# Jimmy2027/MoPoE-MIMIC

Hardware: AMD Instinct MI355X
Metric: samples/sec (higher is better)
Workload: dtype f32; 1 GPU; BASELINE config c2: MoPoE joint-ELBO train step, 3 modalities (PA+Lateral+text) 128x128, class_dim 128, DIM_img 64, DIM_text 128, vocab 3517, batch 64/GPU, fp32 (storage, accumulation and every product; where the launch plan says so the fp32 products are formed on the bf16 matrix pipe from exact three-way splits of both operands -- closer to fp64 than the fp32 MFMA, tests: test_f32_products_on_the; global_batch=64, parallelism=dp1, hip_graph=True, cross_rank_elbo=mean

## Files before the change

mopoe-mimic_amd/csrc/conv_gemm.hip:

```cpp
#include "gemm_common.hpp"

namespace mopoe {

#ifndef GEMM_MIN_WAVES
#define GEMM_MIN_WAVES 3
#endif
#ifndef GEMM_LDS_PAD
#define GEMM_LDS_PAD 4
#endif
constexpr int LDS_PAD = GEMM_LDS_PAD;

struct GemmArgs {
  const float* X;
  const float* W;
  float* Y;
  const float* bias;
  int N, Hx, Wx, Hy, Wy, Ck, Cn, Cin_w, Cout_w;
  int kh, kw, sh, sw, ph, pw;
  int form, w_nk;
  int Hq, Wq;
  long rows_per_phase;
  int vecA, vecB;
  mopoe_bn_ref bn_in;
  mopoe_mask_ref mask;
  double* out_stats;
  mopoe_bn_ref relu_bn;
  const float* xin;
  double* bwd_sums;
  unsigned x_bytes, w_bytes;
  int nsplit;
  float* partial;
  int* counters;
  long rows_total;
  int mix;
  float mix_a, mix_b;
  int xcd_remap;
};

__device__ __forceinline__ float epi_round(const GemmArgs&, float x) { return x; }
struct EpiXinRaw { float4 lo, hi; };
constexpr bool EPI_PREFETCH_XIN = false;
__device__ __forceinline__ EpiXinRaw epi_xin_ld(const GemmArgs& a, long yrow, int ncol, bool ok_hi) {
  const float* p = a.xin + yrow * a.Cn + ncol;
// ... 6 lines not shown
  xi[0] = r.lo.x; xi[1] = r.lo.y; xi[2] = r.lo.z; xi[3] = r.lo.w; xi[4] = r.hi.x; xi[5] = r.hi.y; xi[6] = r.hi.z; xi[7] = r.hi.w;
}
__device__ __forceinline__ void epi_store8(const GemmArgs& a, long yrow, int ncol, bool ok_hi, const float (&v)[8]) {
  float* dst = a.Y + yrow * a.Cn + ncol;
  *reinterpret_cast<float4*>(dst) = make_float4(v[0], v[1], v[2], v[3]);
  if (ok_hi) *reinterpret_cast<float4*>(dst + 4) = make_float4(v[4], v[5], v[6], v[7]);
}


__device__ __forceinline__ float4 bld4(__amdgpu_buffer_rsrc_t srd, unsigned byte_off) {
  const u32x4 v = __builtin_amdgcn_raw_buffer_load_b128(srd, byte_off, 0, 0);
  return make_float4(__uint_as_float(v.x), __uint_as_float(v.y), __uint_as_float(v.z), __uint_as_float(v.w));
}

__device__ __forceinline__ float4 bld4s(__amdgpu_buffer_rsrc_t srd, unsigned byte_off, unsigned s_off) {
  const u32x4 v = __builtin_amdgcn_raw_buffer_load_b128(srd, byte_off, s_off, 0);
  return make_float4(__uint_as_float(v.x), __uint_as_float(v.y), __uint_as_float(v.z), __uint_as_float(v.w));
}

__device__ __forceinline__ float4 ld4(const float* p, int nvalid, bool vec) {
  float4 v = make_float4(0.f, 0.f, 0.f, 0.f);
  if (nvalid >= 4 && vec) {
    v = *reinterpret_cast<const float4*>(p);
  } else {
    if (nvalid > 0) v.x = p[0];
    if (nvalid > 1) v.y = p[1];
    if (nvalid > 2) v.z = p[2];
    if (nvalid > 3) v.w = p[3];
  }
  return v;
}

template <int BM, int BN, int WGM, int WGN, int GBK, bool VEC, int SPEC = 0>
__global__ __launch_bounds__(64 * WGM * WGN, (WGM * WGN == 4 ? GEMM_MIN_WAVES : ((BM / WGM) * (BN / WGN) > 64 * 32 ? 2 : 4)))
void gather_gemm_kernel(const GemmArgs a) {
  static_assert(SPEC == 0 || VEC, "specialised loops exist for the vector path only");
  constexpr int NT = 64 * WGM * WGN;
  static_assert(WGM * WGN == 4 || WGM * WGN == 8, "4 or 8 waves per block");
  constexpr int WM = BM / WGM, WN = BN / WGN;
  constexpr int TI = WM / 32, TJ = WN / 32;
  constexpr int A_LD = BM + LDS_PAD, B_LD = BN + LDS_PAD;
  constexpr int KQ = GBK / 4;
  constexpr int RPP = NT / KQ;
  constexpr int A_PER_THR = BM / RPP;
  static_assert(BM % RPP == 0, "A tile rows must be a multiple of the rows covered per pass");
  constexpr int B_PER_THR_NK = (BN + RPP - 1) / RPP;
  constexpr int N4 = BN / 4;
  constexpr int B_PER_THR_KN = (GBK * N4 + NT - 1) / NT;
  constexpr int B_PER_THR = B_PER_THR_NK > B_PER_THR_KN ? B_PER_THR_NK : B_PER_THR_KN;

  constexpr int STG_LD = WN + 4;
  constexpr int A_FLOATS = 2 * GBK * A_LD, B_FLOATS = 2 * GBK * B_LD;
  constexpr int STG_FLOATS = VEC ? (NT / 64) * 32 * STG_LD : 0;
  constexpr int SMEM_FLOATS = (A_FLOATS + B_FLOATS) > STG_FLOATS ? (A_FLOATS + B_FLOATS) : STG_FLOATS;
  __shared__ __attribute__((aligned(16))) float smem[SMEM_FLOATS];
  __shared__ __attribute__((aligned(16))) float bnS[MAX_BN_C];
  __shared__ __attribute__((aligned(16))) float bnT[MAX_BN_C];
  __shared__ __attribute__((aligned(16))) float epi[5][VEC ? BN : 4];
  __shared__ int s_ticket;
  float* const As0 = smem;
  float* const Bs0 = smem + A_FLOATS;
#define AS_(buf, k, r) As0[((buf) * GBK + (k)) * A_LD + (r)]
#define BS_(buf, k, r) Bs0[((buf) * GBK + (k)) * B_LD + (r)]

  const int tid = threadIdx.x;
  const int lane = tid & 63, wave = tid >> 6;
  const int wm = wave / WGN, wn = wave % WGN;
  unsigned lbx = blockIdx.x, lby = blockIdx.y, lbz = blockIdx.z;
  if (a.xcd_remap) {
    const unsigned inner = gridDim.y * gridDim.z;
    const unsigned sw = xcd_swizzle(blockIdx.x + gridDim.x * (blockIdx.y + gridDim.y * blockIdx.z), gridDim.x * inner);
    lbx = sw / inner;
    const unsigned rem = sw - lbx * inner;
    lby = rem % gridDim.y;
    lbz = rem / gridDim.y;
  }
  const int n0 = lby * BN;
  const int phase = lbz / a.nsplit;
  const int split = lbz - phase * a.nsplit;

  const TapWalk tw = tap_walk(a, phase);
  const int nty = tw.nty, ntx = tw.ntx, ky0 = tw.ky0, kx0 = tw.kx0, kstep_y = tw.kstep_y, kstep_x = tw.kstep_x;
// ... 65 lines not shown
    for (int i = 0; i < B_PER_THR_KN; ++i) {
      const int k = tid / N4 + i * (NT / N4);
      const int n = n0 + (tid % N4) * 4;
      if ((k < GBK) & (n < a.Cn)) voffB[i] = ((unsigned)k * (unsigned)a.Cout_w + (unsigned)n) * 4u;
    }
  } else {
#pragma unroll
    for (int i = 0; i < B_PER_THR_NK; ++i) {
      const int n = n0 + trow + i * RPP;
      if ((trow + i * RPP < BN) & (n < a.Cn)) voffB[i] = ((unsigned)n * (unsigned)a.Cout_w + (unsigned)kq * 4u) * 4u;
    }
  }

  const long nMt = (a.rows_per_phase + BM - 1) / BM;
  for (long mt = lbx; mt < nMt; mt += gridDim.x) {
    const long m0 = mt * BM;

    int rn[A_PER_THR], ry0[A_PER_THR], rx0[A_PER_THR], rbase[A_PER_THR];
    bool rvalid[A_PER_THR];
#pragma unroll
    for (int i = 0; i < A_PER_THR; ++i) {
      const long m = m0 + trow + i * RPP;
      rvalid[i] = m < a.rows_per_phase;
      const unsigned mm = rvalid[i] ? (unsigned)m : 0u;
      const int n = (int)(mm / (unsigned)hw);
      const int rem = (int)(mm - (unsigned)n * (unsigned)hw);
      const int qy = rem / a.Wq, qx = rem - qy * a.Wq;
      rn[i] = n;
      if (a.form == 0) { ry0[i] = qy * a.sh - a.ph; rx0[i] = qx * a.sw - a.pw; }
      else             { ry0[i] = qy + cy;          rx0[i] = qx + cx; }
      rbase[i] = (n * a.Hx + ry0[i]) * a.Wx + rx0[i];
    }

    float4 ra[A_PER_THR], rb[B_PER_THR];
    float4 pend_sc = make_float4(0.f, 0.f, 0.f, 0.f), pend_sh = pend_sc;
    bool pend_ok[A_PER_THR];

    int ld_tap = it_beg / nkc;
    int ld_kc = (it_beg - ld_tap * nkc) * GBK;
    bool tap_dirty = true;
    unsigned offA[A_PER_THR], offW = 0;
    bool okA[A_PER_THR];

    auto load_tiles = [&](int ) {
      if (tap_dirty) {
        const int jy = ld_tap / ntx, jx = ld_tap - jy * ntx;
        const int wtap = (ky0 + kstep_y * jy) * a.kw + (kx0 + kstep_x * jx);
        const int tapoff = dsgn * (jy * a.Wx + jx);
#pragma unroll
        for (int i = 0; i < A_PER_THR; ++i) {
          const int iy = ry0[i] + dsgn * jy, ix = rx0[i] + dsgn * jx;
          okA[i] = rvalid[i] & ((unsigned)iy < (unsigned)a.Hx) & ((unsigned)ix < (unsigned)a.Wx);
          offA[i] = (unsigned)(rbase[i] + tapoff) * (unsigned)a.Ck * 4u;
        }
        offW = (unsigned)wtap * (unsigned)a.Cin_w * (unsigned)a.Cout_w * 4u;
        if (fastk) {
#pragma unroll
          for (int i = 0; i < A_PER_THR; ++i) {
            offA[i] = okA[i] ? offA[i] + (unsigned)kq * 16u : OOB;
            pend_ok[i] = okA[i];
          }
        }
        tap_dirty = false;
      }
      if (fastk) {
        const unsigned sA = (unsigned)ld_kc * 4u;
        const unsigned sB = offW + (w_nk == 0 ? (unsigned)ld_kc * (unsigned)a.Cout_w * 4u : (unsigned)ld_kc * 4u);
        if (xform) {
          pend_sc = *reinterpret_cast<const float4*>(&bnS[ld_kc + kq * 4]);
          pend_sh = *reinterpret_cast<const float4*>(&bnT[ld_kc + kq * 4]);
        }
        if constexpr (VEC) {
#pragma unroll
          for (int i = 0; i < A_PER_THR; ++i) ra[i] = bld4s(srdX, offA[i], sA);
          if (w_nk == 0) {
#pragma unroll
            for (int i = 0; i < B_PER_THR_KN; ++i) rb[i] = bld4s(srdW, voffB[i], sB);
          } else {
#pragma unroll
            for (int i = 0; i < B_PER_THR_NK; ++i) rb[i] = bld4s(srdW, voffB[i], sB);
          }
        }
        ld_kc += GBK;
        if (ld_kc >= nkc * GBK) { ld_kc = 0; ++ld_tap; tap_dirty = true; }
        return;
      }
      const int kc = ld_kc;
      const int ck = kc + kq * 4;
      const int nvk = a.Ck - ck;
      if (xform) {
        const int cks = nvk > 0 ? ck : 0;
        pend_sc = *reinterpret_cast<const float4*>(&bnS[cks]);
        pend_sh = *reinterpret_cast<const float4*>(&bnT[cks]);
      }
#pragma unroll
      for (int i = 0; i < A_PER_THR; ++i) {
        const bool ok = okA[i] & (nvk > 0);
        float4 v;
        if constexpr (VEC) {
          v = bld4(srdX, ok ? offA[i] + (unsigned)ck * 4u : OOB);
        } else {
          v = make_float4(0.f, 0.f, 0.f, 0.f);
          if (ok) v = ld4(a.X + (long)(offA[i] >> 2) + ck, nvk, false);
        }
        pend_ok[i] = ok;
        ra[i] = v;
      }
      if (w_nk == 0) {
#pragma unroll
        for (int i = 0; i < B_PER_THR_KN; ++i) {
          const int k = tid / N4 + i * (NT / N4);
          const int n = n0 + (tid % N4) * 4;
          const int kk = kc + k;
          const bool ok = (k < GBK) & (kk < a.Ck) & (n < a.Cn);
          if constexpr (VEC) {
            rb[i] = bld4(srdW, ok ? offW + ((unsigned)kk * (unsigned)a.Cout_w + (unsigned)n) * 4u : OOB);
          } else {
            float4 v = make_float4(0.f, 0.f, 0.f, 0.f);
            if (ok) v = ld4(a.W + (long)(offW >> 2) + (long)kk * a.Cout_w + n, a.Cn - n, false);
            rb[i] = v;
          }
        }
      } else {
#pragma unroll
        for (int i = 0; i < B_PER_THR_NK; ++i) {
          const int n = n0 + trow + i * RPP;
          const bool ok = (trow + i * RPP < BN) & (n < a.Cn) & (nvk > 0);
          if constexpr (VEC) {
            rb[i] = bld4(srdW, ok ? offW + ((unsigned)n * (unsigned)a.Cout_w + (unsigned)ck) * 4u : OOB);
          } else {
            float4 v = make_float4(0.f, 0.f, 0.f, 0.f);
            if (ok) v = ld4(a.W + (long)(offW >> 2) + (long)n * a.Cout_w + ck, nvk, false);
            rb[i] = v;
          }
        }
      }
      ld_kc += GBK;
      if (ld_kc >= nkc * GBK) { ld_kc = 0; ++ld_tap; tap_dirty = true; }
    };

    auto store_tiles = [&](auto bufc) {
      constexpr int buf = decltype(bufc)::value;
#pragma unroll
      for (int i = 0; i < A_PER_THR; ++i) {
        const int r = trow + i * RPP;
        if (xform) {
          const bool ok = pend_ok[i];
          ra[i].x = ok ? fmaxf(fmaf(ra[i].x, pend_sc.x, pend_sh.x), 0.f) : 0.f;
          ra[i].y = ok ? fmaxf(fmaf(ra[i].y, pend_sc.y, pend_sh.y), 0.f) : 0.f;
          ra[i].z = ok ? fmaxf(fmaf(ra[i].z, pend_sc.z, pend_sh.z), 0.f) : 0.f;
          ra[i].w = ok ? fmaxf(fmaf(ra[i].w, pend_sc.w, pend_sh.w), 0.f) : 0.f;
        }
        AS_(buf, kq * 4 + 0, r) = ra[i].x;
        AS_(buf, kq * 4 + 1, r) = ra[i].y;
        AS_(buf, kq * 4 + 2, r) = ra[i].z;
        AS_(buf, kq * 4 + 3, r) = ra[i].w;
      }
      if (w_nk == 0) {
#pragma unroll
        for (int i = 0; i < B_PER_THR_KN; ++i) {
          const int k = tid / N4 + i * (NT / N4);
          if (k < GBK) *reinterpret_cast<float4*>(&BS_(buf, k, (tid % N4) * 4)) = rb[i];
        }
      } else {
#pragma unroll
        for (int i = 0; i < B_PER_THR_NK; ++i) {
          const int r = trow + i * RPP;
          if (r >= BN) continue;
          BS_(buf, kq * 4 + 0, r) = rb[i].x;
          BS_(buf, kq * 4 + 1, r) = rb[i].y;
          BS_(buf, kq * 4 + 2, r) = rb[i].z;
          BS_(buf, kq * 4 + 3, r) = rb[i].w;
        }
      }
    };

    f32x16 acc[TI][TJ];
#pragma unroll
    for (int i = 0; i < TI; ++i)
#pragma unroll
      for (int j = 0; j < TJ; ++j)
#pragma unroll
        for (int r = 0; r < 16; ++r) acc[i][j][r] = 0.f;

    if (total > 0) {
      load_tiles(it_beg);
      store_tiles(std::integral_constant<int, 0>{});
    }
    __syncthreads();

    auto chunk = [&](int it, auto curc) {
      constexpr int cur = decltype(curc)::value;
      if (it + 1 < total) load_tiles(it_beg + it + 1);
      __builtin_amdgcn_sched_barrier(0);
#ifdef GEMM_SETPRIO
      __builtin_amdgcn_s_setprio(1);
#endif
#pragma unroll
      for (int kk = 0; kk < GBK / 2; ++kk) {
        const int k = kk * 2 + lhi;
        float av[TI], bv[TJ];
#pragma unroll
        for (int i = 0; i < TI; ++i) av[i] = AS_(cur, k, wm * WM + i * 32 + l31);
#pragma unroll
        for (int j = 0; j < TJ; ++j) bv[j] = BS_(cur, k, wn * WN + j * 32 + l31);
#pragma unroll
        for (int i = 0; i < TI; ++i)
#pragma unroll
          for (int j = 0; j < TJ; ++j)
            acc[i][j] = __builtin_amdgcn_mfma_f32_32x32x2f32(av[i], bv[j], acc[i][j], 0, 0, 0);
      }
#ifdef GEMM_SETPRIO
      __builtin_amdgcn_s_setprio(0);
#endif
      if (it + 1 < total) store_tiles(std::integral_constant<int, cur ^ 1>{});
      __syncthreads();
    };
    int it = 0;
    for (; it + 1 < total; it += 2) {
      chunk(it, std::integral_constant<int, 0>{});
      chunk(it + 1, std::integral_constant<int, 1>{});
    }
    if (it < total) chunk(it, std::integral_constant<int, 0>{});

    if constexpr (VEC) {
#include "gemm_epilogue_rows.inc"
    } else {
#include "gemm_epilogue.inc"
    }
  }

  if constexpr (VEC) {
#include "gemm_colstats_rows.inc"
  } else {
#include "gemm_colstats.inc"
  }
#undef AS_
#undef BS_
}

__device__ __forceinline__ float bld1s(__amdgpu_buffer_rsrc_t srd, unsigned byte_off, unsigned s_off) {
  return __uint_as_float(__builtin_amdgcn_raw_buffer_load_b32(srd, byte_off, s_off, 0));
}

template <int WGM, int WGN, int TI, int TJ, int SPEC>
__global__ __launch_bounds__(64 * WGM * WGN, (TI * TJ >= 4 ? 3 : 4)) void direct_gemm_kernel(const GemmArgs a) {
  constexpr int NT = 64 * WGM * WGN;
  constexpr int WM = TI * 32, WN = TJ * 32, BM = WGM * WM, BN = WGN * WN;
  constexpr bool xform = SPEC == 2;
  constexpr int w_nk = SPEC == 3 ? 1 : 0;
  constexpr int KS = 8;

  __shared__ __attribute__((aligned(16))) float bnS[xform ? MAX_BN_C : 4];
  __shared__ __attribute__((aligned(16))) float bnT[xform ? MAX_BN_C : 4];

  const int tid = threadIdx.x;
// ... 202 lines not shown
  __shared__ __attribute__((aligned(16))) float Is[2][BK][I_LD];
  __shared__ __attribute__((aligned(16))) float Js[2][BK][J_LD];
  __shared__ __attribute__((aligned(16))) float bnS[MAX_BN_C];
  __shared__ __attribute__((aligned(16))) float bnT[MAX_BN_C];

  const int tid = threadIdx.x;
  const int lane = tid & 63, wave = tid >> 6;
  const int wi = wave >> 1, wj = wave & 1;
  const unsigned lin = a.xcd_remap ? xcd_swizzle(blockIdx.x + gridDim.x * (blockIdx.y + gridDim.y * blockIdx.z),
                                                 gridDim.x * gridDim.y * gridDim.z)
                                   : blockIdx.x + gridDim.x * (blockIdx.y + gridDim.y * blockIdx.z);
  const unsigned bx = lin % gridDim.x, byz = lin / gridDim.x;
  const unsigned by = byz % gridDim.y, bz = byz / gridDim.y;
  const int it_i = bx / a.nJ, it_j = bx % a.nJ;
  const int i0 = it_i * BI, j0 = it_j * BJ;
  const int tap = by;
  const int ky = tap / a.kw, kx = tap % a.kw;
  const long mbeg = (long)bz * a.chunk;
  const long mend = mbeg + a.chunk < a.Ms ? mbeg + a.chunk : a.Ms;
  const int total = (int)((mend - mbeg + BK - 1) / BK);

  const bool xform = SPEC ? (SPEC == 2) : (a.bn_in.mode != 0);
  const bool fast = SPEC ? true : (VEC && a.fast != 0);
  if (xform) {
    for (int c = tid; c < ((a.Cin + 3) & ~3); c += 256) {
      BnC k = BnC{0.f, 0.f, 0.f, 0.f};
      if (c < a.Cin) k = bn_coef(a.bn_in, c);
      bnS[c] = k.scale;
      bnT[c] = k.shift;
    }
    __syncthreads();
  }

  float4 ri[I_PER_THR], rj[J_PER_THR];
  bool pend_ok[I_PER_THR];
  const int hw = a.Hs * a.Ws;
  const __amdgpu_buffer_rsrc_t srdX = __builtin_amdgcn_make_buffer_rsrc((void*)a.Xs, 0, (int)a.x_bytes, 0x00020000);
  const __amdgpu_buffer_rsrc_t srdD = __builtin_amdgcn_make_buffer_rsrc((void*)a.Dy, 0, (int)a.dy_bytes, 0x00020000);

  static_assert(BI == BJ, "both operand tiles cover the same pixels per thread");
  constexpr int PPP = 256 / I4;
  int pn[I_PER_THR], pqy[I_PER_THR], pqx[I_PER_THR];
  long pm[I_PER_THR];
#pragma unroll
  for (int t = 0; t < I_PER_THR; ++t) {
    pm[t] = mbeg + tid / I4 + t * PPP;
    const unsigned m = (unsigned)(pm[t] < a.Ms ? pm[t] : 0);
    const unsigned n = m / (unsigned)hw;
    const unsigned rem = m - n * (unsigned)hw;
    pn[t] = (int)n; pqy[t] = rem / a.Ws; pqx[t] = rem - pqy[t] * a.Ws;
  }

  float4 sc4 = make_float4(0.f, 0.f, 0.f, 0.f), sh4 = sc4;
  const int ci = i0 + (tid % I4) * 4, cj = j0 + (tid % J4) * 4;
  if (xform) {
    const int cs = ci < a.Cin ? ci : 0;
    sc4 = *reinterpret_cast<const float4*>(&bnS[cs]);
    sh4 = *reinterpret_cast<const float4*>(&bnT[cs]);
  }

  const int rpc = a.Ws >= BK ? 1 : BK / a.Ws;
  const int big_c = a.x_is_big ? a.Cin : a.Cout;
  const unsigned shift_rows = (unsigned)(a.ph * a.Wb + a.pw);
  const unsigned shift_bytes = shift_rows * (unsigned)big_c * 4u;
  const __amdgpu_buffer_rsrc_t srdBig = __builtin_amdgcn_make_buffer_rsrc(
      (void*)((const char*)(a.x_is_big ? a.Xs : a.Dy) - shift_bytes), 0,
      (int)((a.x_is_big ? a.x_bytes : a.dy_bytes) + shift_bytes), 0x00020000);
  int f_ly[I_PER_THR], f_lx[I_PER_THR];
  unsigned f_vbig[I_PER_THR], f_vsmall_i[I_PER_THR], f_vsmall_j[I_PER_THR];
  int f_slot[I_PER_THR];
  int f_n = 0, f_qy = 0, f_qx = 0;
  unsigned f_m0 = 0;
  if (fast) {
#pragma unroll
    for (int t = 0; t < I_PER_THR; ++t) {
      const int p = tid / I4 + t * PPP;
      const int pdy = a.Ws >= BK ? 0 : p / a.Ws, pqx = a.Ws >= BK ? p : p - (p / a.Ws) * a.Ws;
      f_slot[t] = p;
      f_ly[t] = pdy * a.sh + ky - a.ph;
      f_lx[t] = pqx * a.sw + kx - a.pw;
      const unsigned lane_rows = (unsigned)((f_ly[t] + a.ph) * a.Wb + (f_lx[t] + a.pw));
      const int cbig = a.x_is_big ? ci : cj;
      f_vbig[t] = (cbig < big_c) ? (lane_rows * (unsigned)big_c + (unsigned)cbig) * 4u : OOB;
      f_vsmall_i[t] = (ci < a.Cin) ? ((unsigned)p * (unsigned)a.Cin + (unsigned)ci) * 4u : OOB;
      f_vsmall_j[t] = (cj < a.Cout) ? ((unsigned)p * (unsigned)a.Cout + (unsigned)cj) * 4u : OOB;
    }
    const unsigned m0 = (unsigned)mbeg;
    f_m0 = m0;
    f_n = (int)(m0 / (unsigned)hw);
    const unsigned rem = m0 - (unsigned)f_n * (unsigned)hw;
    f_qy = (int)(rem / (unsigned)a.Ws);
    f_qx = (int)(rem - (unsigned)f_qy * (unsigned)a.Ws);
  }

  auto load_tiles = [&](int ) {
    if (fast) {
      if constexpr (VEC) {
        const int nleft = (int)((unsigned)mend - f_m0);
        const int s_by = f_qy * a.sh, s_bx = f_qx * a.sw;
        const unsigned s_big = (unsigned)((f_n * a.Hb + s_by) * a.Wb + s_bx) * (unsigned)big_c * 4u;
        const unsigned s_small_i = f_m0 * (unsigned)a.Cin * 4u, s_small_j = f_m0 * (unsigned)a.Cout * 4u;
#pragma unroll
        for (int t = 0; t < I_PER_THR; ++t) {
          const bool inm = f_slot[t] < nleft;
          const bool inb = ((unsigned)(s_by + f_ly[t]) < (unsigned)a.Hb) & ((unsigned)(s_bx + f_lx[t]) < (unsigned)a.Wb);
          const unsigned vb = (inm & inb) ? f_vbig[t] : OOB;
          if (a.x_is_big) {
            ri[t] = bld4s(srdBig, vb, s_big);
            rj[t] = bld4s(srdD, inm ? f_vsmall_j[t] : OOB, s_small_j);
            pend_ok[t] = (inm & inb) & (ci < a.Cin);
          } else {
            ri[t] = bld4s(srdX, inm ? f_vsmall_i[t] : OOB, s_small_i);
            rj[t] = bld4s(srdBig, vb, s_big);
            pend_ok[t] = inm & (ci < a.Cin);
          }
        }
        f_m0 += BK;
        if (a.Ws >= BK) { f_qx += BK; if (f_qx >= a.Ws) { f_qx = 0; ++f_qy; } }
        else f_qy += rpc;
        if (f_qy >= a.Hs) { f_qy = 0; ++f_n; }
      }
      return;
    }
#pragma unroll
    for (int t = 0; t < I_PER_THR; ++t) {
      const bool inm = pm[t] < mend;
      const int by = pqy[t] * a.sh - a.ph + ky, bx = pqx[t] * a.sw - a.pw + kx;
      const bool inb = ((unsigned)by < (unsigned)a.Hb) & ((unsigned)bx < (unsigned)a.Wb);
      const int srow = (int)pm[t];
      const int brow = (pn[t] * a.Hb + by) * a.Wb + bx;
      const int rowx = a.x_is_big ? brow : srow, rowd = a.x_is_big ? srow : brow;
      const bool okx = inm & (ci < a.Cin) & (a.x_is_big ? inb : true);
      const bool okd = inm & (cj < a.Cout) & (a.x_is_big ? true : inb);
      pend_ok[t] = okx;
      if constexpr (VEC) {
        ri[t] = bld4(srdX, okx ? ((unsigned)rowx * (unsigned)a.Cin + (unsigned)ci) * 4u : OOB);
        rj[t] = bld4(srdD, okd ? ((unsigned)rowd * (unsigned)a.Cout + (unsigned)cj) * 4u : OOB);
      } else {
        float4 v = make_float4(0.f, 0.f, 0.f, 0.f), w = v;
        if (okx) v = ld4(a.Xs + (long)rowx * a.Cin + ci, a.Cin - ci, false);
        if (okd) w = ld4(a.Dy + (long)rowd * a.Cout + cj, a.Cout - cj, false);
        ri[t] = v; rj[t] = w;
      }
      pm[t] += BK;
      pqx[t] += BK;
      if (pqx[t] >= a.Ws) {
        if (a.Ws >= BK) {
          pqx[t] -= a.Ws; ++pqy[t];
        } else {
          const int carry = pqx[t] / a.Ws;
          pqx[t] -= carry * a.Ws; pqy[t] += carry;
        }
        if (pqy[t] >= a.Hs) {
          const int carry = pqy[t] / a.Hs;
          pqy[t] -= carry * a.Hs; pn[t] += carry;
        }
      }
    }
  };

  auto store_tiles = [&](auto bufc) {
    constexpr int buf = decltype(bufc)::value;
#pragma unroll
    for (int t = 0; t < I_PER_THR; ++t) {
      const int p = tid / I4 + t * (256 / I4);
      if (xform) {
        const bool ok = pend_ok[t];
        ri[t].x = ok ? fmaxf(fmaf(ri[t].x, sc4.x, sh4.x), 0.f) : 0.f;
        ri[t].y = ok ? fmaxf(fmaf(ri[t].y, sc4.y, sh4.y), 0.f) : 0.f;
        ri[t].z = ok ? fmaxf(fmaf(ri[t].z, sc4.z, sh4.z), 0.f) : 0.f;
        ri[t].w = ok ? fmaxf(fmaf(ri[t].w, sc4.w, sh4.w), 0.f) : 0.f;
      }
      *reinterpret_cast<float4*>(&Is[buf][p][(tid % I4) * 4]) = ri[t];
    }
#pragma unroll
    for (int t = 0; t < J_PER_THR; ++t) {
      const int p = tid / J4 + t * (256 / J4);
      *reinterpret_cast<float4*>(&Js[buf][p][(tid % J4) * 4]) = rj[t];
    }
  };

  f32x16 acc[TI][TJ];
#pragma unroll
  for (int i = 0; i < TI; ++i)
#pragma unroll
    for (int j = 0; j < TJ; ++j)
#pragma unroll
      for (int r = 0; r < 16; ++r) acc[i][j][r] = 0.f;

  if (total > 0) {
    load_tiles(0);
    store_tiles(std::integral_constant<int, 0>{});
  }
  __syncthreads();

  const int l31 = lane & 31, lhi = lane >> 5;
  auto chunk = [&](int it, auto curc) {
    constexpr int cur = decltype(curc)::value;
    if (it + 1 < total) load_tiles(it + 1);
    __builtin_amdgcn_sched_barrier(0);
#pragma unroll
    for (int kk = 0; kk < BK / 2; ++kk) {
      const int k = kk * 2 + lhi;
      float av[TI], bv[TJ];
#pragma unroll
      for (int i = 0; i < TI; ++i) av[i] = Is[cur][k][wi * WI + i * 32 + l31];
#pragma unroll
      for (int j = 0; j < TJ; ++j) bv[j] = Js[cur][k][wj * WJ + j * 32 + l31];
#pragma unroll
      for (int i = 0; i < TI; ++i)
#pragma unroll
        for (int j = 0; j < TJ; ++j)
          acc[i][j] = __builtin_amdgcn_mfma_f32_32x32x2f32(av[i], bv[j], acc[i][j], 0, 0, 0);
    }
    if (it + 1 < total) store_tiles(std::integral_constant<int, cur ^ 1>{});
    __syncthreads();
  };
  int it = 0;
  for (; it + 1 < total; it += 2) {
    chunk(it, std::integral_constant<int, 0>{});
    chunk(it + 1, std::integral_constant<int, 1>{});
  }
  if (it < total) chunk(it, std::integral_constant<int, 0>{});

#pragma unroll
  for (int j = 0; j < TJ; ++j) {
    const int co = j0 + wj * WJ + j * 32 + l31;
    if (co >= a.Cout) continue;
#pragma unroll
    for (int i = 0; i < TI; ++i) {
#pragma unroll
      for (int r = 0; r < 16; ++r) {
        const int ci = i0 + wi * WI + i * 32 + (r & 3) + 8 * (r >> 2) + 4 * lhi;
        if (ci >= a.Cin) continue;
        float* dst = a.dW + ((long)tap * a.Cin + ci) * a.Cout + co;
        if (a.atomic) unsafeAtomicAdd(dst, acc[i][j][r]);
        else *dst = acc[i][j][r];
      }
    }
  }
}

#ifndef EPI_MAX_BLOCKS_Y
#define EPI_MAX_BLOCKS_Y 256
#endif
__global__ __launch_bounds__(256) void splitk_epilogue_kernel(const GemmArgs a) {
  __shared__ float cs[2][4][64];
  const int tx = threadIdx.x & 63, ty = threadIdx.x >> 6;
  const int n = blockIdx.x * 64 + tx;
  const bool nok = n < a.Cn;
  const bool do_relu_bn = a.relu_bn.mode != 0;
  const float bias = (nok && a.bias) ? a.bias[n] : 0.f;
  BnC rb = {0.f, 0.f, 0.f, 0.f};
  if (nok && do_relu_bn) rb = bn_coef(a.relu_bn, n);
  const long stride = a.rows_total * (long)a.Cn;
  float s1 = 0.f, s2 = 0.f;
// ... 214 lines not shown
```

mopoe-mimic_amd/csrc/gemm_common.hpp:

```cpp
#pragma once
#include <stdlib.h>
#include <algorithm>
#include <initializer_list>
#include <type_traits>

#include "common.hpp"
#include "conv_launch.hpp"

namespace mopoe {

bool edge_supported(const mopoe_conv_geom* g, int C, std::initializer_list<const void*> ptrs);
template <typename T> int edge_expand(const float* scal, const float* W, T* out, const mopoe_conv_geom* g, int C, double* stats, hipStream_t st);
template <typename T> int edge_wgrad(const T* vec, const float* scal, float* dW, const mopoe_conv_geom* g, int C, hipStream_t st, bool dw_is_zero = false);
template <typename T> int edge_reduce(const T* x, const float* W, const float* bias, float* out, const mopoe_conv_geom* g, int C, hipStream_t st);

typedef float f32x16 __attribute__((ext_vector_type(16)));
typedef unsigned int u32x4 __attribute__((ext_vector_type(4)));

constexpr unsigned OOB = 0x80000000u;

struct TapWalk {
  int nty, ntx;
  int ky0, kx0;
  int kstep_y, kstep_x;
  int dsgn;
  int cy, cx;
  int phy, phx;
};
template <typename Args>
__device__ __forceinline__ TapWalk tap_walk(const Args& a, int phase) {
  TapWalk w;
  w.cy = w.cx = w.phy = w.phx = 0;
  if (a.form == 0) {
    w.nty = a.kh; w.ntx = a.kw; w.ky0 = 0; w.kx0 = 0; w.kstep_y = 1; w.kstep_x = 1; w.dsgn = 1;
  } else {
    w.phy = phase / a.sw; w.phx = phase % a.sw;
    const int ry = (w.phy + a.ph) % a.sh, rx = (w.phx + a.pw) % a.sw;
    w.nty = ry < a.kh ? (a.kh - ry + a.sh - 1) / a.sh : 0;
    w.ntx = rx < a.kw ? (a.kw - rx + a.sw - 1) / a.sw : 0;
    w.ky0 = ry; w.kx0 = rx; w.kstep_y = a.sh; w.kstep_x = a.sw; w.dsgn = -1;
    w.cy = (w.phy + a.ph - ry) / a.sh; w.cx = (w.phx + a.pw - rx) / a.sw;
  }
  return w;
}

static inline bool aligned16(const void* p) { return (reinterpret_cast<uintptr_t>(p) & 15) == 0; }
static inline bool xcd_remap_enabled() { static const bool on = !getenv("MOPOE_NO_XCD_REMAP"); return on; }

template <typename Args, typename T, typename TY>
static inline void fill_gather_args(Args& a, const GatherDecision& d, const mopoe_conv_geom* g, const T* X, const T* W, const float* bias, TY* Y,
// ... 50 lines not shown
```

mopoe-mimic_amd/csrc/gemm_glds_common.inc:

```
#pragma once

typedef __attribute__((address_space(3))) void lds_void_t;

template <int... Ns, typename F>
__device__ __forceinline__ void static_for_impl(std::integer_sequence<int, Ns...>, F&& f) { (f(std::integral_constant<int, Ns>{}), ...); }
template <int N, typename F>
__device__ __forceinline__ void static_for(F&& f) { static_for_impl(std::make_integer_sequence<int, N>{}, f); }

template <int N>
__device__ __forceinline__ void wait_vmcnt() {
  static_assert(N >= 0 && N <= 63, "vmcnt is a 6-bit counter");
  if constexpr (N == 0) asm volatile("s_waitcnt vmcnt(0)" ::: "memory");
  else if constexpr (N == 2) asm volatile("s_waitcnt vmcnt(2)" ::: "memory");
  else if constexpr (N == 3) asm volatile("s_waitcnt vmcnt(3)" ::: "memory");
  else if constexpr (N == 4) asm volatile("s_waitcnt vmcnt(4)" ::: "memory");
  else if constexpr (N == 5) asm volatile("s_waitcnt vmcnt(5)" ::: "memory");
  else if constexpr (N == 6) asm volatile("s_waitcnt vmcnt(6)" ::: "memory");
  else if constexpr (N == 7) asm volatile("s_waitcnt vmcnt(7)" ::: "memory");
  else if constexpr (N == 8) asm volatile("s_waitcnt vmcnt(8)" ::: "memory");
  else if constexpr (N == 10) asm volatile("s_waitcnt vmcnt(10)" ::: "memory");
  else if constexpr (N == 12) asm volatile("s_waitcnt vmcnt(12)" ::: "memory");
  else if constexpr (N == 14) asm volatile("s_waitcnt vmcnt(14)" ::: "memory");
  else if constexpr (N == 16) asm volatile("s_waitcnt vmcnt(16)" ::: "memory");
  else if constexpr (N == 24) asm volatile("s_waitcnt vmcnt(24)" ::: "memory");
  else static_assert(N == 0, "add the literal for this count");
}

#if defined(__HIP_DEVICE_COMPILE__)
#define MOPOE_DEVICE_ASM(...) asm volatile(__VA_ARGS__)
#define MOPOE_DEVICE_ASM_PURE(...) asm(__VA_ARGS__)
#else
#define MOPOE_DEVICE_ASM(...) do { } while (0)
#define MOPOE_DEVICE_ASM_PURE(...) do { } while (0)
#endif
__device__ __forceinline__ void lds_dma16(__amdgpu_buffer_rsrc_t srd, unsigned char* lds_dst, unsigned voff, unsigned soff) {
#if defined(__HIP_DEVICE_COMPILE__)
  __builtin_amdgcn_raw_ptr_buffer_load_lds(srd, (lds_void_t*)lds_dst, 16, voff, soff, 0, 0);
#endif
}

// ... 11 lines not shown
```

Measured before the change: 6680 samples/sec.

## Add multi-stage register prefetch ring to gather and weight-grad GEMM kernels

Adds a compile-time register ring of depth D to the conv gather GEMM and its weight-gradient kernel, so global loads are issued several K-chunks ahead of their LDS store instead of one. The main loop is restructured with a prologue that fills the ring, a steady state, and a drain tail, and the minimum-waves launch bound is lowered for ring variants. The aim is to hide global memory latency in the specialised 4-wave BN=64 tiles. In exchange it uses more VGPRs and lowers occupancy, and the weight-grad ring defaults to depth 1, so that kernel keeps the old schedule.

Measured after the change: 6723 samples/sec (median of 6 runs). No clear change (+0.6%).

```diff
diff --git a/mopoe-mimic_amd/csrc/conv_gemm.hip b/mopoe-mimic_amd/csrc/conv_gemm.hip
--- a/mopoe-mimic_amd/csrc/conv_gemm.hip
+++ b/mopoe-mimic_amd/csrc/conv_gemm.hip
@@ -9,6 +9,30 @@
 #define GEMM_LDS_PAD 4
 #endif
 constexpr int LDS_PAD = GEMM_LDS_PAD;
+
+#ifndef GEMM_RING_T2
+#define GEMM_RING_T2 3
+#endif
+#ifndef GEMM_RING_T4
+#define GEMM_RING_T4 1
+#endif
+#ifndef GEMM_RING_T5
+#define GEMM_RING_T5 2
+#endif
+#ifndef GEMM_RING_T6
+#define GEMM_RING_T6 1
+#endif
+#ifndef GEMM_RING_W2
+#define GEMM_RING_W2 1
+#endif
+#ifndef GEMM_RING_MIN_WAVES
+#define GEMM_RING_MIN_WAVES 2
+#endif
+template <int BM, int BN, int WAVES, int GBK, int SPEC>
+constexpr int gather_ring_depth() {
+  if (WAVES != 4 || BN != 64 || SPEC == 0) return 1;
+  return BM == 64 ? (GBK == 16 ? GEMM_RING_T2 : GEMM_RING_T5) : (GBK == 16 ? GEMM_RING_T4 : GEMM_RING_T6);
+}
 
 struct GemmArgs {
   const float* X;
@@ -81,7 +105,8 @@
 }
 
 template <int BM, int BN, int WGM, int WGN, int GBK, bool VEC, int SPEC = 0>
-__global__ __launch_bounds__(64 * WGM * WGN, (WGM * WGN == 4 ? GEMM_MIN_WAVES : ((BM / WGM) * (BN / WGN) > 64 * 32 ? 2 : 4)))
+__global__ __launch_bounds__(64 * WGM * WGN, (WGM * WGN == 4 ? (gather_ring_depth<BM, BN, WGM * WGN, GBK, SPEC>() > 1 ? GEMM_RING_MIN_WAVES : GEMM_MIN_WAVES)
+                                                               : ((BM / WGM) * (BN / WGN) > 64 * 32 ? 2 : 4)))
 void gather_gemm_kernel(const GemmArgs a) {
   static_assert(SPEC == 0 || VEC, "specialised loops exist for the vector path only");
   constexpr int NT = 64 * WGM * WGN;
@@ -97,6 +122,8 @@
   constexpr int N4 = BN / 4;
   constexpr int B_PER_THR_KN = (GBK * N4 + NT - 1) / NT;
   constexpr int B_PER_THR = B_PER_THR_NK > B_PER_THR_KN ? B_PER_THR_NK : B_PER_THR_KN;
+  constexpr int D = gather_ring_depth<BM, BN, WGM * WGN, GBK, SPEC>();
+  static_assert(D >= 1 && D <= 4, "ring depth");
 
   constexpr int STG_LD = WN + 4;
   constexpr int A_FLOATS = 2 * GBK * A_LD, B_FLOATS = 2 * GBK * B_LD;
@@ -228,9 +255,11 @@
       rbase[i] = (n * a.Hx + ry0[i]) * a.Wx + rx0[i];
     }
 
-    float4 ra[A_PER_THR], rb[B_PER_THR];
-    float4 pend_sc = make_float4(0.f, 0.f, 0.f, 0.f), pend_sh = pend_sc;
-    bool pend_ok[A_PER_THR];
+    float4 ra[D][A_PER_THR], rb[D][B_PER_THR];
+    float4 pend_sc[D], pend_sh[D];
+#pragma unroll
+    for (int s = 0; s < D; ++s) pend_sc[s] = pend_sh[s] = make_float4(0.f, 0.f, 0.f, 0.f);
+    bool pend_ok[D][A_PER_THR];
 
     int ld_tap = it_beg / nkc;
     int ld_kc = (it_beg - ld_tap * nkc) * GBK;
@@ -238,7 +267,8 @@
     unsigned offA[A_PER_THR], offW = 0;
     bool okA[A_PER_THR];
 
-    auto load_tiles = [&](int ) {
+    auto load_tiles = [&](auto setc) {
+      constexpr int set = decltype(setc)::value;
       if (tap_dirty) {
         const int jy = ld_tap / ntx, jx = ld_tap - jy * ntx;
         const int wtap = (ky0 + kstep_y * jy) * a.kw + (kx0 + kstep_x * jx);
@@ -254,27 +284,31 @@
 #pragma unroll
           for (int i = 0; i < A_PER_THR; ++i) {
             offA[i] = okA[i] ? offA[i] + (unsigned)kq * 16u : OOB;
-            pend_ok[i] = okA[i];
+            if constexpr (D == 1) pend_ok[set][i] = okA[i];
           }
         }
         tap_dirty = false;
       }
       if (fastk) {
+        if constexpr (D > 1) {
+#pragma unroll
+          for (int i = 0; i < A_PER_THR; ++i) pend_ok[set][i] = okA[i];
+        }
         const unsigned sA = (unsigned)ld_kc * 4u;
         const unsigned sB = offW + (w_nk == 0 ? (unsigned)ld_kc * (unsigned)a.Cout_w * 4u : (unsigned)ld_kc * 4u);
         if (xform) {
-          pend_sc = *reinterpret_cast<const float4*>(&bnS[ld_kc + kq * 4]);
-          pend_sh = *reinterpret_cast<const float4*>(&bnT[ld_kc + kq * 4]);
+          pend_sc[set] = *reinterpret_cast<const float4*>(&bnS[ld_kc + kq * 4]);
+          pend_sh[set] = *reinterpret_cast<const float4*>(&bnT[ld_kc + kq * 4]);
         }
         if constexpr (VEC) {
 #pragma unroll
-          for (int i = 0; i < A_PER_THR; ++i) ra[i] = bld4s(srdX, offA[i], sA);
+          for (int i = 0; i < A_PER_THR; ++i) ra[set][i] = bld4s(srdX, offA[i], sA);
           if (w_nk == 0) {
 #pragma unroll
-            for (int i = 0; i < B_PER_THR_KN; ++i) rb[i] = bld4s(srdW, voffB[i], sB);
+            for (int i = 0; i < B_PER_THR_KN; ++i) rb[set][i] = bld4s(srdW, voffB[i], sB);
           } else {
 #pragma unroll
-            for (int i = 0; i < B_PER_THR_NK; ++i) rb[i] = bld4s(srdW, voffB[i], sB);
+            for (int i = 0; i < B_PER_THR_NK; ++i) rb[set][i] = bld4s(srdW, voffB[i], sB);
           }
         }
         ld_kc += GBK;
@@ -286,8 +320,8 @@
       const int nvk = a.Ck - ck;
       if (xform) {
         const int cks = nvk > 0 ? ck : 0;
-        pend_sc = *reinterpret_cast<const float4*>(&bnS[cks]);
-        pend_sh = *reinterpret_cast<const float4*>(&bnT[cks]);
+        pend_sc[set] = *reinterpret_cast<const float4*>(&bnS[cks]);
+        pend_sh[set] = *reinterpret_cast<const float4*>(&bnT[cks]);
       }
 #pragma unroll
       for (int i = 0; i < A_PER_THR; ++i) {
@@ -299,8 +333,8 @@
           v = make_float4(0.f, 0.f, 0.f, 0.f);
           if (ok) v = ld4(a.X + (long)(offA[i] >> 2) + ck, nvk, false);
         }
-        pend_ok[i] = ok;
-        ra[i] = v;
+        pend_ok[set][i] = ok;
+        ra[set][i] = v;
       }
       if (w_nk == 0) {
 #pragma unroll
@@ -310,11 +344,11 @@
           const int kk = kc + k;
           const bool ok = (k < GBK) & (kk < a.Ck) & (n < a.Cn);
           if constexpr (VEC) {
-            rb[i] = bld4(srdW, ok ? offW + ((unsigned)kk * (unsigned)a.Cout_w + (unsigned)n) * 4u : OOB);
+            rb[set][i] = bld4(srdW, ok ? offW + ((unsigned)kk * (unsigned)a.Cout_w + (unsigned)n) * 4u : OOB);
           } else {
             float4 v = make_float4(0.f, 0.f, 0.f, 0.f);
             if (ok) v = ld4(a.W + (long)(offW >> 2) + (long)kk * a.Cout_w + n, a.Cn - n, false);
-            rb[i] = v;
+            rb[set][i] = v;
           }
         }
       } else {
@@ -323,11 +357,11 @@
           const int n = n0 + trow + i * RPP;
           const bool ok = (trow + i * RPP < BN) & (n < a.Cn) & (nvk > 0);
           if constexpr (VEC) {
-            rb[i] = bld4(srdW, ok ? offW + ((unsigned)n * (unsigned)a.Cout_w + (unsigned)ck) * 4u : OOB);
+            rb[set][i] = bld4(srdW, ok ? offW + ((unsigned)n * (unsigned)a.Cout_w + (unsigned)ck) * 4u : OOB);
           } else {
             float4 v = make_float4(0.f, 0.f, 0.f, 0.f);
             if (ok) v = ld4(a.W + (long)(offW >> 2) + (long)n * a.Cout_w + ck, nvk, false);
-            rb[i] = v;
+            rb[set][i] = v;
           }
         }
       }
@@ -335,38 +369,38 @@
       if (ld_kc >= nkc * GBK) { ld_kc = 0; ++ld_tap; tap_dirty = true; }
     };
 
-    auto store_tiles = [&](auto bufc) {
-      constexpr int buf = decltype(bufc)::value;
+    auto store_tiles = [&](auto bufc, auto setc) {
+      constexpr int buf = decltype(bufc)::value, set = decltype(setc)::value;
 #pragma unroll
       for (int i = 0; i < A_PER_THR; ++i) {
         const int r = trow + i * RPP;
         if (xform) {
-          const bool ok = pend_ok[i];
-          ra[i].x = ok ? fmaxf(fmaf(ra[i].x, pend_sc.x, pend_sh.x), 0.f) : 0.f;
-          ra[i].y = ok ? fmaxf(fmaf(ra[i].y, pend_sc.y, pend_sh.y), 0.f) : 0.f;
-          ra[i].z = ok ? fmaxf(fmaf(ra[i].z, pend_sc.z, pend_sh.z), 0.f) : 0.f;
-          ra[i].w = ok ? fmaxf(fmaf(ra[i].w, pend_sc.w, pend_sh.w), 0.f) : 0.f;
-        }
-        AS_(buf, kq * 4 + 0, r) = ra[i].x;
-        AS_(buf, kq * 4 + 1, r) = ra[i].y;
-        AS_(buf, kq * 4 + 2, r) = ra[i].z;
-        AS_(buf, kq * 4 + 3, r) = ra[i].w;
+          const bool ok = pend_ok[set][i];
+          ra[set][i].x = ok ? fmaxf(fmaf(ra[set][i].x, pend_sc[set].x, pend_sh[set].x), 0.f) : 0.f;
+          ra[set][i].y = ok ? fmaxf(fmaf(ra[set][i].y, pend_sc[set].y, pend_sh[set].y), 0.f) : 0.f;
+          ra[set][i].z = ok ? fmaxf(fmaf(ra[set][i].z, pend_sc[set].z, pend_sh[set].z), 0.f) : 0.f;
+          ra[set][i].w = ok ? fmaxf(fmaf(ra[set][i].w, pend_sc[set].w, pend_sh[set].w), 0.f) : 0.f;
+        }
+        AS_(buf, kq * 4 + 0, r) = ra[set][i].x;
+        AS_(buf, kq * 4 + 1, r) = ra[set][i].y;
+        AS_(buf, kq * 4 + 2, r) = ra[set][i].z;
+        AS_(buf, kq * 4 + 3, r) = ra[set][i].w;
       }
       if (w_nk == 0) {
 #pragma unroll
         for (int i = 0; i < B_PER_THR_KN; ++i) {
           const int k = tid / N4 + i * (NT / N4);
-          if (k < GBK) *reinterpret_cast<float4*>(&BS_(buf, k, (tid % N4) * 4)) = rb[i];
+          if (k < GBK) *reinterpret_cast<float4*>(&BS_(buf, k, (tid % N4) * 4)) = rb[set][i];
         }
       } else {
 #pragma unroll
         for (int i = 0; i < B_PER_THR_NK; ++i) {
           const int r = trow + i * RPP;
           if (r >= BN) continue;
-          BS_(buf, kq * 4 + 0, r) = rb[i].x;
-          BS_(buf, kq * 4 + 1, r) = rb[i].y;
-          BS_(buf, kq * 4 + 2, r) = rb[i].z;
-          BS_(buf, kq * 4 + 3, r) = rb[i].w;
+          BS_(buf, kq * 4 + 0, r) = rb[set][i].x;
+          BS_(buf, kq * 4 + 1, r) = rb[set][i].y;
+          BS_(buf, kq * 4 + 2, r) = rb[set][i].z;
+          BS_(buf, kq * 4 + 3, r) = rb[set][i].w;
         }
       }
     };
@@ -379,15 +413,19 @@
 #pragma unroll
         for (int r = 0; r < 16; ++r) acc[i][j][r] = 0.f;
 
-    if (total > 0) {
-      load_tiles(it_beg);
-      store_tiles(std::integral_constant<int, 0>{});
-    }
-    __syncthreads();
-
-    auto chunk = [&](int it, auto curc) {
-      constexpr int cur = decltype(curc)::value;
-      if (it + 1 < total) load_tiles(it_beg + it + 1);
+    using I0 = std::integral_constant<int, 0>;
+    using I1 = std::integral_constant<int, 1>;
+    if constexpr (D == 1) {
+      if (total > 0) {
+        load_tiles(I0{});
+        store_tiles(I0{}, I0{});
+      }
+      __syncthreads();
+    }
+
+    auto chunk = [&](int it, auto curc, auto setc, auto modec) {
+      constexpr int cur = decltype(curc)::value, set = decltype(setc)::value, MODE = decltype(modec)::value;
+      if (MODE == 0 ? it + 1 < total : MODE == 1) load_tiles(setc);
       __builtin_amdgcn_sched_barrier(0);
 #ifdef GEMM_SETPRIO
       __builtin_amdgcn_s_setprio(1);
@@ -409,15 +447,59 @@
 #ifdef GEMM_SETPRIO
       __builtin_amdgcn_s_setprio(0);
 #endif
-      if (it + 1 < total) store_tiles(std::integral_constant<int, cur ^ 1>{});
+      if (MODE == 0 ? it + 1 < total : MODE != 3)
+        store_tiles(std::integral_constant<int, cur ^ 1>{}, std::integral_constant<int, (set + 1) % D>{});
       __syncthreads();
     };
-    int it = 0;
-    for (; it + 1 < total; it += 2) {
-      chunk(it, std::integral_constant<int, 0>{});
-      chunk(it + 1, std::integral_constant<int, 1>{});
-    }
-    if (it < total) chunk(it, std::integral_constant<int, 0>{});
+    if constexpr (D == 1) {
+      int it = 0;
+      for (; it + 1 < total; it += 2) {
+        chunk(it, I0{}, I0{}, I0{});
+        chunk(it + 1, I1{}, I0{}, I0{});
+      }
+      if (it < total) chunk(it, I0{}, I0{}, I0{});
+    } else {
+      auto drain = [&](auto uc, auto rc) {
+        constexpr int U = decltype(uc)::value, R = decltype(rc)::value;
+        static_for<R>([&](auto jc) {
+          constexpr int j = decltype(jc)::value;
+          chunk(0, std::integral_constant<int, (U + j) % 2>{}, std::integral_constant<int, (U + j) % D>{},
+                std::integral_constant<int, (j + 1 < R ? 2 : 3)>{});
+        });
+      };
+      if (total >= D) {
+        static_for<D>([&](auto sc) { load_tiles(sc); });
+        store_tiles(I0{}, I0{});
+        __syncthreads();
+        constexpr int UNR = D % 2 == 0 ? D : 2 * D;
+        bool drained = false;
+        for (int it = 0; !drained; it += UNR) {
+          static_for<UNR>([&](auto uc) {
+            constexpr int u = decltype(uc)::value;
+            if (drained) return;
+            if (it + u + D < total) {
+              chunk(it + u, std::integral_constant<int, u % 2>{}, std::integral_constant<int, u % D>{}, I1{});
+            } else {
+              drain(uc, std::integral_constant<int, D>{});
+              drained = true;
+            }
+          });
+        }
+      } else {
+        static_for<D - 1>([&](auto tc) {
+          constexpr int T = decltype(tc)::value + 1;
+          if (total == T) {
+            static_for<T>([&](auto sc) { load_tiles(sc); });
+            store_tiles(I0{}, I0{});
+          }
+        });
+        __syncthreads();
+        static_for<D - 1>([&](auto tc) {
+          constexpr int T = decltype(tc)::value + 1;
+          if (total == T) drain(I0{}, std::integral_constant<int, T>{});
+        });
+      }
+    }
 
     if constexpr (VEC) {
 #include "gemm_epilogue_rows.inc"
@@ -686,8 +768,10 @@
     __syncthreads();
   }
 
-  float4 ri[I_PER_THR], rj[J_PER_THR];
-  bool pend_ok[I_PER_THR];
+  constexpr int D = (BI == 64 && SPEC != 0) ? GEMM_RING_W2 : 1;
+  static_assert(D >= 1 && D <= 4, "ring depth");
+  float4 ri[D][I_PER_THR], rj[D][J_PER_THR];
+  bool pend_ok[D][I_PER_THR];
   const int hw = a.Hs * a.Ws;
   const __amdgpu_buffer_rsrc_t srdX = __builtin_amdgcn_make_buffer_rsrc((void*)a.Xs, 0, (int)a.x_bytes, 0x00020000);
   const __amdgpu_buffer_rsrc_t srdD = __builtin_amdgcn_make_buffer_rsrc((void*)a.Dy, 0, (int)a.dy_bytes, 0x00020000);
@@ -747,7 +831,8 @@
     f_qx = (int)(rem - (unsigned)f_qy * (unsigned)a.Ws);
   }
 
-  auto load_tiles = [&](int ) {
+  auto load_tiles = [&](auto setc) {
+    constexpr int set = decltype(setc)::value;
     if (fast) {
       if constexpr (VEC) {
         const int nleft = (int)((unsigned)mend - f_m0);
@@ -760,13 +845,13 @@
           const bool inb = ((unsigned)(s_by + f_ly[t]) < (unsigned)a.Hb) & ((unsigned)(s_bx + f_lx[t]) < (unsigned)a.Wb);
           const unsigned vb = (inm & inb) ? f_vbig[t] : OOB;
           if (a.x_is_big) {
-            ri[t] = bld4s(srdBig, vb, s_big);
-            rj[t] = bld4s(srdD, inm ? f_vsmall_j[t] : OOB, s_small_j);
-            pend_ok[t] = (inm & inb) & (ci < a.Cin);
+            ri[set][t] = bld4s(srdBig, vb, s_big);
+            rj[set][t] = bld4s(srdD, inm ? f_vsmall_j[t] : OOB, s_small_j);
+            pend_ok[set][t] = (inm & inb) & (ci < a.Cin);
           } else {
-            ri[t] = bld4s(srdX, inm ? f_vsmall_i[t] : OOB, s_small_i);
-            rj[t] = bld4s(srdBig, vb, s_big);
-            pend_ok[t] = inm & (ci < a.Cin);
+            ri[set][t] = bld4s(srdX, inm ? f_vsmall_i[t] : OOB, s_small_i);
+            rj[set][t] = bld4s(srdBig, vb, s_big);
+            pend_ok[set][t] = inm & (ci < a.Cin);
           }
         }
         f_m0 += BK;
@@ -786,15 +871,15 @@
       const int rowx = a.x_is_big ? brow : srow, rowd = a.x_is_big ? srow : brow;
       const bool okx = inm & (ci < a.Cin) & (a.x_is_big ? inb : true);
       const bool okd = inm & (cj < a.Cout) & (a.x_is_big ? true : inb);
-      pend_ok[t] = okx;
+      pend_ok[set][t] = okx;
       if constexpr (VEC) {
-        ri[t] = bld4(srdX, okx ? ((unsigned)rowx * (unsigned)a.Cin + (unsigned)ci) * 4u : OOB);
-        rj[t] = bld4(srdD, okd ? ((unsigned)rowd * (unsigned)a.Cout + (unsigned)cj) * 4u : OOB);
+        ri[set][t] = bld4(srdX, okx ? ((unsigned)rowx * (unsigned)a.Cin + (unsigned)ci) * 4u : OOB);
+        rj[set][t] = bld4(srdD, okd ? ((unsigned)rowd * (unsigned)a.Cout + (unsigned)cj) * 4u : OOB);
       } else {
         float4 v = make_float4(0.f, 0.f, 0.f, 0.f), w = v;
         if (okx) v = ld4(a.Xs + (long)rowx * a.Cin + ci, a.Cin - ci, false);
         if (okd) w = ld4(a.Dy + (long)rowd * a.Cout + cj, a.Cout - cj, false);
-        ri[t] = v; rj[t] = w;
+        ri[set][t] = v; rj[set][t] = w;
       }
       pm[t] += BK;
       pqx[t] += BK;
@@ -813,24 +898,24 @@
     }
   };
 
-  auto store_tiles = [&](auto bufc) {
-    constexpr int buf = decltype(bufc)::value;
+  auto store_tiles = [&](auto bufc, auto setc) {
+    constexpr int buf = decltype(bufc)::value, set = decltype(setc)::value;
 #pragma unroll
     for (int t = 0; t < I_PER_THR; ++t) {
       const int p = tid / I4 + t * (256 / I4);
       if (xform) {
-        const bool ok = pend_ok[t];
-        ri[t].x = ok ? fmaxf(fmaf(ri[t].x, sc4.x, sh4.x), 0.f) : 0.f;
-        ri[t].y = ok ? fmaxf(fmaf(ri[t].y, sc4.y, sh4.y), 0.f) : 0.f;
-        ri[t].z = ok ? fmaxf(fmaf(ri[t].z, sc4.z, sh4.z), 0.f) : 0.f;
-        ri[t].w = ok ? fmaxf(fmaf(ri[t].w, sc4.w, sh4.w), 0.f) : 0.f;
-      }
-      *reinterpret_cast<float4*>(&Is[buf][p][(tid % I4) * 4]) = ri[t];
+        const bool ok = pend_ok[set][t];
+        ri[set][t].x = ok ? fmaxf(fmaf(ri[set][t].x, sc4.x, sh4.x), 0.f) : 0.f;
+        ri[set][t].y = ok ? fmaxf(fmaf(ri[set][t].y, sc4.y, sh4.y), 0.f) : 0.f;
+        ri[set][t].z = ok ? fmaxf(fmaf(ri[set][t].z, sc4.z, sh4.z), 0.f) : 0.f;
+        ri[set][t].w = ok ? fmaxf(fmaf(ri[set][t].w, sc4.w, sh4.w), 0.f) : 0.f;
+      }
+      *reinterpret_cast<float4*>(&Is[buf][p][(tid % I4) * 4]) = ri[set][t];
     }
 #pragma unroll
     for (int t = 0; t < J_PER_THR; ++t) {
       const int p = tid / J4 + t * (256 / J4);
-      *reinterpret_cast<float4*>(&Js[buf][p][(tid % J4) * 4]) = rj[t];
+      *reinterpret_cast<float4*>(&Js[buf][p][(tid % J4) * 4]) = rj[set][t];
     }
   };
 
@@ -842,16 +927,20 @@
 #pragma unroll
       for (int r = 0; r < 16; ++r) acc[i][j][r] = 0.f;
 
-  if (total > 0) {
-    load_tiles(0);
-    store_tiles(std::integral_constant<int, 0>{});
-  }
-  __syncthreads();
+  using I0 = std::integral_constant<int, 0>;
+  using I1 = std::integral_constant<int, 1>;
+  if constexpr (D == 1) {
+    if (total > 0) {
+      load_tiles(I0{});
+      store_tiles(I0{}, I0{});
+    }
+    __syncthreads();
+  }
 
   const int l31 = lane & 31, lhi = lane >> 5;
-  auto chunk = [&](int it, auto curc) {
-    constexpr int cur = decltype(curc)::value;
-    if (it + 1 < total) load_tiles(it + 1);
+  auto chunk = [&](int it, auto curc, auto setc, auto modec) {
+    constexpr int cur = decltype(curc)::value, set = decltype(setc)::value, MODE = decltype(modec)::value;
+    if (MODE == 0 ? it + 1 < total : MODE == 1) load_tiles(setc);
     __builtin_amdgcn_sched_barrier(0);
 #pragma unroll
     for (int kk = 0; kk < BK / 2; ++kk) {
@@ -867,15 +956,59 @@
         for (int j = 0; j < TJ; ++j)
           acc[i][j] = __builtin_amdgcn_mfma_f32_32x32x2f32(av[i], bv[j], acc[i][j], 0, 0, 0);
     }
-    if (it + 1 < total) store_tiles(std::integral_constant<int, cur ^ 1>{});
+    if (MODE == 0 ? it + 1 < total : MODE != 3)
+      store_tiles(std::integral_constant<int, cur ^ 1>{}, std::integral_constant<int, (set + 1) % D>{});
     __syncthreads();
   };
-  int it = 0;
-  for (; it + 1 < total; it += 2) {
-    chunk(it, std::integral_constant<int, 0>{});
-    chunk(it + 1, std::integral_constant<int, 1>{});
-  }
-  if (it < total) chunk(it, std::integral_constant<int, 0>{});
+  if constexpr (D == 1) {
+    int it = 0;
+    for (; it + 1 < total; it += 2) {
+      chunk(it, I0{}, I0{}, I0{});
+      chunk(it + 1, I1{}, I0{}, I0{});
+    }
+    if (it < total) chunk(it, I0{}, I0{}, I0{});
+  } else {
+    auto drain = [&](auto uc, auto rc) {
+      constexpr int U = decltype(uc)::value, R = decltype(rc)::value;
+      static_for<R>([&](auto jc) {
+        constexpr int j = decltype(jc)::value;
+        chunk(0, std::integral_constant<int, (U + j) % 2>{}, std::integral_constant<int, (U + j) % D>{},
+              std::integral_constant<int, (j + 1 < R ? 2 : 3)>{});
+      });
+    };
+    if (total >= D) {
+      static_for<D>([&](auto sc) { load_tiles(sc); });
+      store_tiles(I0{}, I0{});
+      __syncthreads();
+      constexpr int UNR = D % 2 == 0 ? D : 2 * D;
+      bool drained = false;
+      for (int it = 0; !drained; it += UNR) {
+        static_for<UNR>([&](auto uc) {
+          constexpr int u = decltype(uc)::value;
+          if (drained) return;
+          if (it + u + D < total) {
+            chunk(it + u, std::integral_constant<int, u % 2>{}, std::integral_constant<int, u % D>{}, I1{});
+          } else {
+            drain(uc, std::integral_constant<int, D>{});
+            drained = true;
+          }
+        });
+      }
+    } else {
+      static_for<D - 1>([&](auto tc) {
+        constexpr int T = decltype(tc)::value + 1;
+        if (total == T) {
+          static_for<T>([&](auto sc) { load_tiles(sc); });
+          store_tiles(I0{}, I0{});
+        }
+      });
+      __syncthreads();
+      static_for<D - 1>([&](auto tc) {
+        constexpr int T = decltype(tc)::value + 1;
+        if (total == T) drain(I0{}, std::integral_constant<int, T>{});
+      });
+    }
+  }
 
 #pragma unroll
   for (int j = 0; j < TJ; ++j) {
diff --git a/mopoe-mimic_amd/csrc/gemm_common.hpp b/mopoe-mimic_amd/csrc/gemm_common.hpp
--- a/mopoe-mimic_amd/csrc/gemm_common.hpp
+++ b/mopoe-mimic_amd/csrc/gemm_common.hpp
@@ -3,6 +3,7 @@
 #include <algorithm>
 #include <initializer_list>
 #include <type_traits>
+#include <utility>
 
 #include "common.hpp"
 #include "conv_launch.hpp"
@@ -16,6 +17,11 @@
 
 typedef float f32x16 __attribute__((ext_vector_type(16)));
 typedef unsigned int u32x4 __attribute__((ext_vector_type(4)));
+
+template <int... Ns, typename F>
+__device__ __forceinline__ void static_for_impl(std::integer_sequence<int, Ns...>, F&& f) { (f(std::integral_constant<int, Ns>{}), ...); }
+template <int N, typename F>
+__device__ __forceinline__ void static_for(F&& f) { static_for_impl(std::make_integer_sequence<int, N>{}, f); }
 
 constexpr unsigned OOB = 0x80000000u;
 
diff --git a/mopoe-mimic_amd/csrc/gemm_glds_common.inc b/mopoe-mimic_amd/csrc/gemm_glds_common.inc
--- a/mopoe-mimic_amd/csrc/gemm_glds_common.inc
+++ b/mopoe-mimic_amd/csrc/gemm_glds_common.inc
@@ -1,11 +1,6 @@
 #pragma once
 
 typedef __attribute__((address_space(3))) void lds_void_t;
-
-template <int... Ns, typename F>
-__device__ __forceinline__ void static_for_impl(std::integer_sequence<int, Ns...>, F&& f) { (f(std::integral_constant<int, Ns>{}), ...); }
-template <int N, typename F>
-__device__ __forceinline__ void static_for(F&& f) { static_for_impl(std::make_integer_sequence<int, N>{}, f); }
 
 template <int N>
 __device__ __forceinline__ void wait_vmcnt() {
```
